# kubeflow/Code-Intelligence

Hardware: NVIDIA H100
Metric: issues/sec to 2400-d @ seq_len 512 batch 256 (higher is better)
Workload: dtype bf16

## Files before the change

code_intelligence_b200/_lib.py:

```python
from __future__ import annotations

import ctypes as C
import os
import subprocess
from pathlib import Path

_PKG = Path(__file__).resolve().parent
LIB_PATH = _PKG / "libissue_emb_b200.so"

IE_OK, IE_ERR_INVALID, IE_ERR_CUDA, IE_ERR_OOM, IE_ERR_STATE, IE_ERR_TOKEN = 0, -1, -2, -3, -4, -5
IE_FLAG_DEVICE_PTRS = 1
IE_MAX_BATCH = 3072
IE_CFG_ACCURATE_GATES, IE_CFG_FP32, IE_CFG_F32_GX = 1, 2, 4
IE_KNN_COSINE, IE_KNN_EUCLIDEAN = 0, 1


class ie_config(C.Structure):
    _fields_ = [("n_layers", C.c_int32), ("emb_sz", C.c_int32), ("n_hid", C.c_int32), ("vocab_sz", C.c_int32),
                ("pad_idx", C.c_int32), ("device", C.c_int32), ("flags", C.c_int32)]


PROTOTYPES = {
    "ie_version": (C.c_int, []),
    "ie_last_error": (C.c_char_p, []),
    "ie_encoder_create": (C.c_int, [C.POINTER(ie_config), C.POINTER(C.c_void_p)]),
    "ie_encoder_destroy": (None, [C.c_void_p]),
    "ie_encoder_load_embedding": (C.c_int, [C.c_void_p, C.c_void_p]),
    "ie_encoder_load_layer": (C.c_int, [C.c_void_p, C.c_int32, C.c_void_p, C.c_void_p, C.c_void_p, C.c_void_p]),
    "ie_encoder_encode": (C.c_int, [C.c_void_p, C.c_void_p, C.c_void_p, C.c_int32, C.c_int32, C.c_void_p, C.c_int32,
                                    C.c_void_p]),
    "ie_encoder_raw_features": (C.c_int, [C.c_void_p, C.c_void_p, C.c_int32, C.c_int32, C.c_void_p, C.c_int32,
                                          C.c_void_p]),
    "ie_encoder_launch_count": (C.c_int64, [C.c_void_p]),
    "ie_encoder_max_batch": (C.c_int32, [C.c_void_p]),
    "ie_encoder_check_errors": (C.c_int, [C.c_void_p]),
    "ie_encoder_last_phase_ms": (C.c_int, [C.c_void_p, C.c_void_p, C.c_int32]),
    "ie_encoder_last_phase_mhz": (C.c_int, [C.c_void_p, C.c_void_p, C.c_int32]),
    "ie_debug_seq_trace": (C.c_int64, [C.c_void_p, C.c_int32, C.c_void_p, C.c_int64]),
    "ie_mlp_create": (C.c_int, [C.c_int32, C.POINTER(C.c_int32), C.c_int32, C.POINTER(C.c_void_p)]),
    "ie_mlp_load_layer": (C.c_int, [C.c_void_p, C.c_int32, C.c_void_p, C.c_void_p]),
    "ie_mlp_predict_proba": (C.c_int, [C.c_void_p, C.c_void_p, C.c_int32, C.c_void_p, C.c_int32, C.c_void_p]),
    "ie_mlp_destroy": (None, [C.c_void_p]),
    "ie_pr_thresholds": (C.c_int, [C.c_void_p, C.c_void_p, C.c_int32, C.c_int32, C.c_double, C.c_double, C.c_void_p,
                                   C.c_void_p, C.c_void_p, C.c_int32, C.c_int32, C.c_void_p]),
    "ie_debug_gemm": (C.c_int, [C.c_void_p, C.c_void_p, C.c_void_p, C.c_int32, C.c_int32, C.c_int32, C.c_int32,
                                C.c_void_p, C.c_int32]),
    "ie_debug_gemm_ex": (C.c_int, [C.c_void_p, C.c_void_p, C.c_void_p, C.c_int32, C.c_int32, C.c_int32, C.c_int32,
                                   C.c_int32, C.c_int32, C.c_void_p, C.c_int32]),
    "ie_debug_gemm_frag": (C.c_int, [C.c_void_p, C.c_void_p, C.c_void_p, C.c_int32, C.c_int32, C.c_int32, C.c_int32,
                                     C.c_int32, C.c_void_p, C.c_int32]),
    "ie_debug_epilogue_layout": (C.c_int64, [C.c_int32, C.c_void_p, C.c_int64, C.c_void_p, C.c_void_p]),
    "ie_debug_layer_states": (C.c_int, [C.c_void_p, C.c_int32, C.c_void_p, C.c_int32, C.c_int32, C.c_void_p, C.c_int32,
                                        C.c_void_p]),
    "ie_knn_create": (C.c_int, [C.c_int32, C.c_int32, C.c_int32, C.POINTER(C.c_void_p)]),
    "ie_knn_destroy": (None, [C.c_void_p]),
    "ie_knn_add": (C.c_int, [C.c_void_p, C.c_void_p, C.c_int64, C.c_int32, C.c_void_p]),
    "ie_knn_search": (C.c_int, [C.c_void_p, C.c_void_p, C.c_int32, C.c_int32, C.c_void_p, C.c_void_p, C.c_int32,
                                C.c_void_p]),
    "ie_knn_check_errors": (C.c_int, [C.c_void_p]),
    "ie_debug_knn_shortlist": (C.c_int, [C.c_void_p, C.c_void_p, C.c_int32, C.c_int32, C.c_void_p, C.c_void_p]),
}

_lib = None


def build(verbose: bool = False) -> Path:
    r = subprocess.run(["make", "-C", str(_PKG / "csrc"), "-j8"], capture_output=True, text=True)
    if verbose or r.returncode != 0:
        print(r.stdout[-4000:])
        print(r.stderr[-4000:])
    if r.returncode != 0:
        raise RuntimeError("building libissue_emb_b200.so failed")
    return LIB_PATH


def load() -> C.CDLL:
    global _lib
    if _lib is not None:
        return _lib
    if not LIB_PATH.exists():
        if os.environ.get("IE_B200_NO_AUTOBUILD"):
            raise ImportError(f"{LIB_PATH} is missing (run `python -c 'import __graft_entry__ as g; g.build()'`)")
        build()
    lib = C.CDLL(str(LIB_PATH))
    for name, (res, args) in PROTOTYPES.items():
        fn = getattr(lib, name)
        fn.restype = res
        fn.argtypes = args
    _lib = lib
    return lib


def _debug_gemm(a, b, bias=None, act: int = 0, out_type: int = 0, segs: int = 1, device: int = 0):
    import numpy as np
    a = np.ascontiguousarray(a, dtype=np.float32)
    b = np.ascontiguousarray(b, dtype=np.float32)
    (M, K), N = a.shape, b.shape[0]
    if b.shape[1] != K:
        raise ValueError(f"a {a.shape} and b {b.shape} disagree on K")
    bias_p = None
    if bias is not None:
        bias = np.ascontiguousarray(bias, dtype=np.float32)
        if bias.shape != (N,):
            raise ValueError(f"bias {bias.shape} != ({N},)")
        bias_p = bias.ctypes.data
    d = np.empty((M, N), dtype=np.float32)
    check(load().ie_debug_gemm_ex(a.ctypes.data, b.ctypes.data, bias_p, M, N, K, act, out_type, segs, d.ctypes.data,
                                  device))
    return d


def check(rc: int) -> None:
    if rc == IE_OK:
        return
    msg = (load().ie_last_error() or b"").decode("utf-8", "replace")
    if rc in (IE_ERR_INVALID, IE_ERR_TOKEN):
        raise ValueError(msg)
    if rc == IE_ERR_OOM:
        raise RuntimeError("CUDA out of memory. " + msg)
    raise RuntimeError(msg)
```

code_intelligence_b200/csrc/api.cu:

```cuda
#include <algorithm>
#include <cmath>
#include <cstdarg>
#include <cstdio>
#include <cstdlib>
#include <cstring>
#include <mutex>
#include <string>
#include <vector>

#include <cuda_fp16.h>

#include "../../include/issue_emb_b200.h"
#include "kernels.h"

namespace {

thread_local std::string g_last_error;

int fail(int code, const char* fmt, ...) {
  char buf[512];
  va_list ap;
  va_start(ap, fmt);
  vsnprintf(buf, sizeof(buf), fmt, ap);
  va_end(ap);
// ... 934 lines not shown
  if (n16 >= 240 && n16 % 240 == 0) bn = 240;
  else if (n16 >= 128) bn = 128;
  else bn = n16;
  if (frag) bn = 256;
  const int n_pad = static_cast<int>(round_up(N, bn));
  const int ld = segs == 3 ? 2 * k_pad : k_pad;
  const size_t elt = out_type == 0 ? 4 : 2;
  DevBuf fa, fb, ba, bb, dd, db;
  cudaStream_t s = nullptr;
  CK(fa.reserve(static_cast<size_t>(M) * K * 4));
  CK(fb.reserve(static_cast<size_t>(N) * K * 4));
  CK(ba.reserve(static_cast<size_t>(m_pad) * ld * 2, true));
  CK(bb.reserve(static_cast<size_t>(n_pad) * ld * 2, true));
  CK(dd.reserve(static_cast<size_t>(m_pad) * n_pad * elt));
  CK(cudaMemcpy(fa.p, a, static_cast<size_t>(M) * K * 4, cudaMemcpyHostToDevice));
  CK(cudaMemcpy(fb.p, b, static_cast<size_t>(N) * K * 4, cudaMemcpyHostToDevice));
  const int lo_off = segs == 3 ? k_pad : 0;
  CK(ie::launch_convert_rows(fa.as<float>(), K, K, nullptr, M, ba.as<__nv_bfloat16>(), ld, lo_off, s));
  CK(ie::launch_convert_rows(fb.as<float>(), K, K, nullptr, N, bb.as<__nv_bfloat16>(), ld, lo_off, s));
  if (bias) {
    std::vector<float> bp(n_pad, 0.0f);
    if (frag) {
      for (int n = 0; n < N; ++n) bp[n / 256 * 256 + ie::frag_index(n % 256, 4)] = bias[n];
    } else {
      std::copy(bias, bias + N, bp.begin());
    }
    CK(db.reserve(n_pad * 4));
    CK(cudaMemcpy(db.p, bp.data(), n_pad * 4, cudaMemcpyHostToDevice));
  }
  ie::GemmArgs g{};
  g.a = ba.as<__nv_bfloat16>(); g.lda = ld;
  g.b = bb.as<__nv_bfloat16>(); g.ldb = ld;
  g.d = dd.p; g.ldd = n_pad;
  g.bias = bias ? db.as<float>() : nullptr;
  g.m_pad = m_pad; g.n_pad = n_pad; g.k_pad = k_pad;
  g.m_store = M; g.n_store = n_pad; g.bn = bn; g.act = act; g.out_bf16 = out_type; g.num_sms = sms; g.segs = segs;
  g.frag = frag ? 1 : 0;
  CK(ie::launch_gemm_bf16(g, s));
  if (frag) {
    std::vector<uint8_t> raw(static_cast<size_t>(M) * n_pad * elt);
    CK(cudaMemcpy(raw.data(), dd.p, raw.size(), cudaMemcpyDeviceToHost));
    for (size_t r = 0; r < static_cast<size_t>(M); ++r)
      for (int n = 0; n < N; ++n) {
        const size_t src = r * n_pad + n / 256 * 256 + ie::frag_index(n % 256, static_cast<int>(elt));
        if (out_type == 0) {
          std::memcpy(d + r * N + n, raw.data() + src * 4, 4);
        } else {
          __half_raw h;
          std::memcpy(&h.x, raw.data() + src * 2, 2);
          d[r * N + n] = __half2float(__half(h));
        }
      }
  } else if (out_type == 0) {
    CK(cudaMemcpy2D(d, static_cast<size_t>(N) * 4, dd.p, static_cast<size_t>(n_pad) * 4, static_cast<size_t>(N) * 4, M,
                    cudaMemcpyDeviceToHost));
  } else {
    std::vector<uint16_t> h16(static_cast<size_t>(M) * N);
    CK(cudaMemcpy2D(h16.data(), static_cast<size_t>(N) * 2, dd.p, static_cast<size_t>(n_pad) * 2, static_cast<size_t>(N) * 2,
                    M, cudaMemcpyDeviceToHost));
    for (size_t i = 0; i < h16.size(); ++i) {
      if (out_type == 1) {
        const uint32_t bits = static_cast<uint32_t>(h16[i]) << 16;
        std::memcpy(d + i, &bits, 4);
      } else {
        __half_raw r;
        r.x = h16[i];
        d[i] = __half2float(__half(r));
      }
    }
  }
  return IE_OK;
}

int ie_debug_gemm_ex(const float* a, const float* b, const float* bias, int32_t M, int32_t N, int32_t K, int32_t act,
                     int32_t out_type, int32_t segs, float* d, int32_t device) {
  return debug_gemm(a, b, bias, M, N, K, act, out_type, segs, d, device, false);
}

int ie_debug_gemm_frag(const float* a, const float* b, const float* bias, int32_t M, int32_t N, int32_t K, int32_t out_type,
                       int32_t segs, float* d, int32_t device) {
  return debug_gemm(a, b, bias, M, N, K, 0, out_type, segs, d, device, true);
}

int64_t ie_debug_epilogue_layout(int32_t out_units, int32_t* perm, int64_t cap, int32_t* frag2, int32_t* frag4) {
  if (out_units < 1) return fail(IE_ERR_INVALID, "out_units=%d must be >= 1", out_units);
  Layer L;
  L.out = out_units;
  L.out_pad = static_cast<int>(round_up(out_units, 64));
  const std::vector<int> p = slice_perm(L);
  if (perm != nullptr && cap >= static_cast<int64_t>(p.size())) std::copy(p.begin(), p.end(), perm);
  for (int c = 0; c < 256; ++c) {
    if (frag2 != nullptr) frag2[c] = ie::frag_index(c, 2);
    if (frag4 != nullptr) frag4[c] = ie::frag_index(c, 4);
  }
  return static_cast<int64_t>(p.size());
}

int ie_debug_gemm(const float* a, const float* b, const float* bias, int32_t M, int32_t N, int32_t K, int32_t act,
                  float* d, int32_t device) {
  return ie_debug_gemm_ex(a, b, bias, M, N, K, act, 0, 1, d, device);
}

}

struct ie_knn {
  int dim = 0, metric = IE_KNN_COSINE, device = 0, num_sms = 132;
  int k_pad = 0;
  long long n = 0, cap = 0;
  DevBuf xf;
  DevBuf xs;
  DevBuf col;
  DevBuf center;
  double c2 = 0.0;
  bool centred = false;
  DevBuf partial, qf, qs, rowt, cand, cnt, outd, outi, err;
  cudaStream_t own_stream = nullptr;
  cudaStream_t last_stream = nullptr;
  cudaEvent_t done_ev = nullptr;
  bool has_done = false;
  std::mutex mu;
};

namespace {

int knn_begin(ie_knn* h, bool dev, void* stream, cudaStream_t* s) {
  CK(cudaSetDevice(h->device));
  *s = (stream || dev) ? static_cast<cudaStream_t>(stream) : h->own_stream;
  if (h->has_done && *s != h->last_stream) CK(cudaStreamWaitEvent(*s, h->done_ev, 0));
  return IE_OK;
}

int knn_end(ie_knn* h, cudaStream_t s) {
  CK(cudaEventRecord(h->done_ev, s));
  h->last_stream = s;
  h->has_done = true;
  return IE_OK;
}

int knn_grow(DevBuf& b, size_t bytes, size_t keep, cudaStream_t s) {
  if (bytes <= b.cap) return IE_OK;
  DevBuf nb;
  CK(nb.reserve(bytes));
  if (keep) {
    CK(cudaMemcpyAsync(nb.p, b.p, keep, cudaMemcpyDeviceToDevice, s));
    CK(cudaStreamSynchronize(s));
  }
  b = std::move(nb);
  return IE_OK;
}

int knn_check_rows(const float* x, long long rows, int dim, const char* what) {
  for (long long r = 0; r < rows; ++r) {
    const float* v = x + r * dim;
    double s = 0.0;
    for (int i = 0; i < dim; ++i) {
      if (!std::isfinite(v[i]))
        return fail(IE_ERR_INVALID, "%s[%lld][%d] = %g is not finite", what, r, i, static_cast<double>(v[i]));
      s += static_cast<double>(v[i]) * v[i];
    }
    if (s > 0.0 && (s < ie::kKnnNormMin * ie::kKnnNormMin || s > ie::kKnnNormMax * ie::kKnnNormMax))
      return fail(IE_ERR_INVALID, "%s row %lld has norm %g, outside the index's range [2^-48, 2^48] (0 is allowed)",
                  what, r, std::sqrt(s));
  }
  return IE_OK;
}

// ... 194 lines not shown
```

code_intelligence_b200/csrc/gemm.cu:

```cuda
#include "gemm_kernel.cuh"

namespace ie {


cudaError_t launch_gemm_bf16(const GemmArgs& g, cudaStream_t stream) {
  if (g.m_pad % kBlockM || g.k_pad % kBlockK || g.bn % 16 || g.bn < 16 || g.bn > 256 || g.n_pad % g.bn ||
      g.n_store % 16 || g.ldd % 2)
    return cudaErrorInvalidValue;
  CUtensorMap tmA, tmB;
  const int segs = g.segs == 3 ? 3 : 1;
  const uint64_t k_inner = static_cast<uint64_t>(segs == 3 ? 2 : 1) * g.k_pad;
  const long long spin_limit = g.spin_limit > 0 ? g.spin_limit : kSpinLimitDefault;
  cudaError_t e = make_tmap_bf16_2d(&tmA, g.a, k_inner, g.m_pad, g.lda, kBlockK, kBlockM);
  if (e != cudaSuccess) return e;
  e = make_tmap_bf16_2d(&tmB, g.b, k_inner, g.n_pad, g.ldb, kBlockK, kBlockN);
  if (e != cudaSuccess) return e;

  const size_t smem = 1024 + static_cast<size_t>(kGemmStages) * kGemmStageBytes + 2 * kGemmStages * 8 + 32;
  const int num_m_blocks = g.m_pad / kBlockM;
  const int num_n_blocks = (g.n_pad + kBlockN - 1) / kBlockN;
  const int num_k_blocks = g.k_pad / kBlockK;
  const int num_tiles = num_m_blocks * num_n_blocks;
  const int sms = g.num_sms > 0 ? g.num_sms : 132;
  const int grid = num_tiles < sms ? num_tiles : sms;
  const int panel = 16;

#define IE_LAUNCH(OUT, ACT, FRAG)                                                                                  \
  do {                                                                                                             \
    auto kfn = gemm_bf16_kernel<OUT, ACT, FRAG>;                                                                       \
    e = cudaFuncSetAttribute(kfn, cudaFuncAttributeMaxDynamicSharedMemorySize, static_cast<int>(smem));            \
    if (e != cudaSuccess) return e;                                                                                \
    kfn<<<grid, kGemmThreads, smem, stream>>>(tmA, tmB, reinterpret_cast<OUT*>(g.d), g.bias, g.m_store, g.n_store, \
                                              g.ldd, num_m_blocks, num_n_blocks, num_k_blocks, panel, segs,        \
                                              g.k_pad, g.abort_flag, spin_limit, g.diag, DenseEpi{});              \
  } while (0)

  if (g.frag) {
    if (g.act != 0 || g.out_bf16 == 1 || g.bias == nullptr || g.n_store % kBlockN || g.n_store != g.n_pad ||
        (g.ldd * (g.out_bf16 == 2 ? 2 : 4)) % 16)
      return cudaErrorInvalidValue;
    if (g.out_bf16 == 2) IE_LAUNCH(__half, 0, true);
    else IE_LAUNCH(float, 0, true);
  } else if (g.out_bf16 == 2) {
    if (g.act != 0) return cudaErrorInvalidValue;
    IE_LAUNCH(__half, 0, false);
  } else if (g.out_bf16) {
    if (g.act == 0) IE_LAUNCH(__nv_bfloat16, 0, false);
    else if (g.act == 1) IE_LAUNCH(__nv_bfloat16, 1, false);
    else IE_LAUNCH(__nv_bfloat16, 2, false);
  } else {
    if (g.act == 0) IE_LAUNCH(float, 0, false);
    else if (g.act == 1) IE_LAUNCH(float, 1, false);
    else IE_LAUNCH(float, 2, false);
  }
#undef IE_LAUNCH
  return cudaGetLastError();
}

}
```

code_intelligence_b200/csrc/gemm_kernel.cuh:

```cuda
#pragma once
#include <cuda_fp16.h>
#include <type_traits>

#include "kernels.h"
#include "ptx.cuh"

namespace ie {

struct DenseEpi {
  static constexpr bool kSliced = false;
  static constexpr uint64_t kHintA = kEvictNormal;
  static constexpr uint64_t kHintB = kEvictLast;
  struct State {};
};

namespace {

__device__ __forceinline__ uint32_t pack_f16x2(float lo, float hi) {
  const __half2 v = __floats2half2_rn(lo, hi);
  return *reinterpret_cast<const uint32_t*>(&v);
}

constexpr int kBlockM = 128;
constexpr int kBlockN = 256;
constexpr int kBlockK = 64;
constexpr int kGemmThreads = 384;
constexpr int kGemmStages = 4;
constexpr uint32_t kABytes = kBlockM * kBlockK * 2;
constexpr uint32_t kBBytes = kBlockN * kBlockK * 2;
constexpr uint32_t kGemmStageBytes = kABytes + kBBytes;

template <typename OutT, int ACT, bool FRAG, typename Epi = DenseEpi>
__global__ void __launch_bounds__(kGemmThreads, 1)
gemm_bf16_kernel(const __grid_constant__ CUtensorMap tmA, const __grid_constant__ CUtensorMap tmB, OutT* __restrict__ D,
                 const float* __restrict__ bias, int m_store, int n_store, long long ldd, int num_m_blocks,
                 int num_n_blocks, int num_k_blocks, int panel, int segs, int k_pad, unsigned* abort_flag,
                 long long spin_limit, long long* diag, const __grid_constant__ Epi epi) {
  extern __shared__ uint8_t smem_raw[];
  const uint32_t raw = smem_u32(smem_raw);
  uint8_t* smem = smem_raw + ((1024u - (raw & 1023u)) & 1023u);

  uint64_t* full_bar = reinterpret_cast<uint64_t*>(smem + kGemmStages * kGemmStageBytes);
  uint64_t* empty_bar = full_bar + kGemmStages;
  uint32_t* abort_s = reinterpret_cast<uint32_t*>(empty_bar + kGemmStages);
  const Abort ab{abort_s, abort_flag, spin_limit};
  const int nkt = num_k_blocks * segs;

  const int warp = threadIdx.x >> 5;
  const int lane = threadIdx.x & 31;

  if (warp == 0 && lane == 0) {
    tma_prefetch_desc(&tmA);
    tma_prefetch_desc(&tmB);
    if (diag != nullptr && blockIdx.x == 0) {
      unsigned long long g;
      asm volatile("mov.u64 %0, %%globaltimer;" : "=l"(g));
      diag[0] = clock64();
      diag[1] = static_cast<long long>(g);
    }
  }
  if (warp == 1 && lane == 0) {
    for (int s = 0; s < kGemmStages; ++s) {
      mbar_init(&full_bar[s], 1);
      mbar_init(&empty_bar[s], 2);
    }
    *abort_s = 0;
    fence_barrier_init();
  }
  __syncthreads();

  int num_tiles = num_m_blocks * num_n_blocks;
  if constexpr (Epi::kSliced) num_tiles = epi.num_tiles();
  const int panel_tiles = panel * num_n_blocks;
  int first_tile = blockIdx.x;
  if constexpr (Epi::kSliced) first_tile = epi.first_tile(blockIdx.x);
  auto next_tile = [&](int tile) {
    if constexpr (Epi::kSliced) return epi.next_tile(tile, gridDim.x, num_n_blocks);
    else return tile + static_cast<int>(gridDim.x);
  };
  auto decode = [&](int tile, int& m_blk, int& n_blk) {
    if constexpr (Epi::kSliced) {
      epi.decode(tile, num_m_blocks, m_blk, n_blk);
      return;
    }
    const int p = tile / panel_tiles;
    const int r = tile - p * panel_tiles;
    const int m0 = p * panel;
    const int mcnt = min(panel, num_m_blocks - m0);
    n_blk = r / mcnt;
    m_blk = m0 + (r - n_blk * mcnt);
  };

  if (warp < 4) {
    if (warp == 0 && lane == 0) {
      int stage = 0;
      uint32_t phase = 0;
      for (int tile = first_tile; tile < num_tiles && !aborted(ab); tile = next_tile(tile)) {
        int m_blk, n_blk;
        decode(tile, m_blk, n_blk);
        for (int kb = 0; kb < nkt; ++kb) {
          const int seg = kb / num_k_blocks, r = kb - seg * num_k_blocks;
          mbar_wait(&empty_bar[stage], phase ^ 1, ab);
          uint8_t* sa = smem + static_cast<size_t>(stage) * kGemmStageBytes;
          mbar_arrive_expect_tx(&full_bar[stage], kGemmStageBytes);
          tma_load_2d(sa, &tmA, &full_bar[stage], (seg == 1 ? k_pad : 0) + r * kBlockK, m_blk * kBlockM, Epi::kHintA);
          tma_load_2d(sa + kABytes, &tmB, &full_bar[stage], (seg == 2 ? k_pad : 0) + r * kBlockK, n_blk * kBlockN,
                      Epi::kHintB);
          if (++stage == kGemmStages) { stage = 0; phase ^= 1; }
        }
      }
    }
  } else {
    const int wg = (warp - 4) >> 2;
    const int q = lane & 3;
    const int rbase = wg * 64 + (warp & 3) * 16 + (lane >> 2);
    const uint32_t smem_base = smem_u32(smem);
    const bool signal = (threadIdx.x & 127) == 0;
    int stage = 0;
    uint32_t phase = 0;
    float d[128];
    typename Epi::State st{};
    for (int tile = first_tile; tile < num_tiles; tile = next_tile(tile)) {
      int m_blk, n_blk;
      decode(tile, m_blk, n_blk);
      int prev = -1;
      for (int kb = 0; kb < nkt; ++kb) {
        mbar_wait(&full_bar[stage], phase, ab);
        const uint32_t sa = smem_base + stage * kGemmStageBytes;
        const uint64_t da = wgmma_desc_sw128(sa + wg * (kABytes / 2));
        const uint64_t db = wgmma_desc_sw128(sa + kABytes);
        wgmma_fence();
#pragma unroll
        for (int k = 0; k < kBlockK / 16; ++k) wgmma_m64n256k16(d, da + 2 * k, db + 2 * k, (kb | k) != 0);
        wgmma_commit();
        if (prev >= 0) {
          wgmma_wait<1>();
          if (signal) mbar_arrive(&empty_bar[prev]);
        }
        prev = stage;
        if (++stage == kGemmStages) { stage = 0; phase ^= 1; }
      }
      wgmma_wait<0>();
      wgmma_fence_regs(d);
      if (signal && prev >= 0) mbar_arrive(&empty_bar[prev]);
      if constexpr (Epi::kSliced) {
        epi.tile(d, m_blk, n_blk, wg * 64 + (warp & 3) * 16, lane, st);
        continue;
      }
      if constexpr (FRAG) {
        constexpr int kPer = 16 / static_cast<int>(sizeof(OutT));
        const float4* bq = reinterpret_cast<const float4*>(bias) + n_blk * (kBlockN / 4) + q;
        OutT* drow[2];
#pragma unroll
        for (int hr = 0; hr < 2; ++hr)
          drow[hr] = D + static_cast<long long>(m_blk * kBlockM + rbase + 8 * hr) * ldd + n_blk * kBlockN + q * kPer;
#pragma unroll
        for (int k = 0; k < 64 / kPer; ++k) {
          float4 b[kPer / 4];
#pragma unroll
          for (int i = 0; i < kPer / 4; ++i) b[i] = __ldg(bq + 4 * (k * (kPer / 4) + i));
#pragma unroll
          for (int hr = 0; hr < 2; ++hr) {
            if (m_blk * kBlockM + rbase + 8 * hr >= m_store) continue;
            float x[kPer];
#pragma unroll
            for (int i = 0; i < kPer / 4; ++i) {
              const int m = k * (kPer / 4) + i;
              x[4 * i + 0] = d[8 * m + 2 * hr] + b[i].x;
              x[4 * i + 1] = d[8 * m + 2 * hr + 1] + b[i].y;
              x[4 * i + 2] = d[8 * m + 4 + 2 * hr] + b[i].z;
              x[4 * i + 3] = d[8 * m + 4 + 2 * hr + 1] + b[i].w;
            }
            uint4 v;
            if constexpr (sizeof(OutT) == 4) {
              v = make_uint4(__float_as_uint(x[0]), __float_as_uint(x[1]), __float_as_uint(x[2]), __float_as_uint(x[3]));
            } else {
              v = make_uint4(pack_f16x2(x[0], x[1]), pack_f16x2(x[2], x[3]), pack_f16x2(x[4], x[5]), pack_f16x2(x[6], x[7]));
            }
            *reinterpret_cast<uint4*>(drow[hr] + 4 * k * kPer) = v;
          }
        }
        continue;
      }
#pragma unroll
      for (int hr = 0; hr < 2; ++hr) {
        const int row = m_blk * kBlockM + rbase + 8 * hr;
        if (row >= m_store) continue;
        OutT* drow = D + static_cast<long long>(row) * ldd;
#pragma unroll
        for (int jg = 0; jg < kBlockN / 8; ++jg) {
          const int n = n_blk * kBlockN + 8 * jg + 2 * q;
          if (n < n_store) {
            float x0 = d[4 * jg + 2 * hr], x1 = d[4 * jg + 2 * hr + 1];
            if (bias != nullptr) {
              const float2 b2 = __ldg(reinterpret_cast<const float2*>(bias + n));
              x0 += b2.x;
              x1 += b2.y;
            }
            if (ACT == 1) { x0 = fmaxf(x0, 0.0f); x1 = fmaxf(x1, 0.0f); }
            if (ACT == 2) { x0 = sigmoid_acc(x0); x1 = sigmoid_acc(x1); }
            if constexpr (sizeof(OutT) == 4) {
              *reinterpret_cast<float2*>(drow + n) = make_float2(x0, x1);
            } else if constexpr (std::is_same<OutT, __half>::value) {
              *reinterpret_cast<uint32_t*>(drow + n) = pack_f16x2(x0, x1);
            } else {
              *reinterpret_cast<uint32_t*>(drow + n) = pack_bf16x2(x0, x1);
            }
          }
        }
      }
    }
    if constexpr (Epi::kSliced) epi.finish(wg * 64 + (warp & 3) * 16, lane, st);
  }

  __syncwarp();
  if (diag != nullptr && threadIdx.x == 128 && blockIdx.x == 0) {
    unsigned long long g;
    asm volatile("mov.u64 %0, %%globaltimer;" : "=l"(g));
    diag[2] = clock64();
    diag[3] = static_cast<long long>(g);
  }
}

}

}
```

code_intelligence_b200/csrc/kernels.h:

```cpp
#pragma once
#include <cuda.h>
#include <cuda_bf16.h>
#include <cuda_runtime.h>
#include <stddef.h>
#include <stdint.h>

namespace ie {

cudaError_t make_tmap_bf16_2d(CUtensorMap* out, const void* base, uint64_t inner, uint64_t rows, uint64_t ld,
                              uint32_t box_inner, uint32_t box_rows);

__host__ __device__ inline int frag_index(int c, int elem_bytes) {
  const int q = (c & 7) >> 1;
  const int ix = 4 * (c >> 4) + 2 * ((c >> 3) & 1) + (c & 1);
  const int per_chunk = 16 / elem_bytes;
  return (ix / per_chunk * 4 + q) * per_chunk + ix % per_chunk;
}

struct GemmArgs {
  const __nv_bfloat16* a;
  const __nv_bfloat16* b;
  void* d;
  const float* bias;
  int m_pad, n_pad, k_pad;
  long long lda, ldb, ldd;
  int m_store, n_store;
  int bn;
  int act;
  int out_bf16;
  int num_sms;
  int segs;
  unsigned* abort_flag;
  long long spin_limit;
  long long* diag;
  int frag;
};
cudaError_t launch_gemm_bf16(const GemmArgs& g, cudaStream_t stream);

constexpr int kMaxBatches = 12;
struct LstmLayerArgs {
  CUtensorMap tm_h;
  CUtensorMap tm_w;
  CUtensorMap tm_h64;
  CUtensorMap tm_x;
  int pre_nkb;
  const float* bias;
  int mc;
  int mc_ctas;
  const void* gx;
  const int* tok;
  float* c;
  __nv_bfloat16* y;
  float* raw;
  float* pool_sum;
  float* pool_max;
  float* pool_last;
  const int* lengths;
  unsigned* step_done;
  unsigned* abort_flag;
  long long spin_limit;
  int T, t0, T_total;
  int single_step;
  int t_step;
  int ng;
  int u, n_cta, out_pad, kh_pad;
  long long ldy, raw_ld;
  int gate_mode, gx_bf16, segs;
  int num_sms, check_only, cooperative;
  int fault;
  long long* trace;
  int trace_items;
  long long* diag;
};
cudaError_t launch_lstm_layer(const LstmLayerArgs& a, cudaStream_t stream);
int lstm_layer_ctas(const LstmLayerArgs& a);
int lstm_layer_max_ctas();

cudaError_t launch_embed_gather(const int64_t* ids, int B, int T, int b_pad, const __nv_bfloat16* emb, int vocab,
                                int e_pad, __nv_bfloat16* x0, long long ldx, int pad_idx, int* err_flag, int t0, int Tc,
                                cudaStream_t stream);
cudaError_t launch_prep_lengths(const int* lengths_in, int B, int T, int b_pad, int* lengths_out, int* err_flag,
                                cudaStream_t stream);
cudaError_t launch_tokens_time_major(const int64_t* ids, int B, int T, int b_pad, int vocab, int pad_idx, int* tok,
                                     int* err_flag, cudaStream_t stream);
cudaError_t launch_pool_finalize(const float* pool_sum, const float* pool_max, const float* pool_last,
                                 const int* lengths, int B, int e, int out_pad, float* out, cudaStream_t stream);
cudaError_t launch_convert_rows(const float* src, long long ld_src, int cols, const int* perm, int rows_dst,
                                __nv_bfloat16* dst, long long ld_dst, int lo_off, cudaStream_t stream);
cudaError_t launch_fill_f32(float* p, size_t n, float v, cudaStream_t stream);

constexpr int kPrMaxSamples = 16384;
cudaError_t launch_pr_thresholds(const float* scores, const uint8_t* truth, int n, int n_labels, double p_thr,
                                 double r_thr, float* out_thr, double* out_prec, double* out_rec, cudaStream_t stream);

constexpr int kKnnCap = 512;
constexpr int kKnnMergeMax = 16384;
constexpr int kKnnExtra = 32;
constexpr double kKnnNormMin = 0x1p-48, kKnnNormMax = 0x1p48;
size_t knn_center_workspace(int D);
cudaError_t launch_knn_center(const float* x, long long n, int D, int k_pad, double* partial, float* center,
                              cudaStream_t stream);
cudaError_t launch_knn_prep(const float* src, long long rows, long long rows_pad, int D, int k_pad, const float* center,
                            double c2, int mode, __nv_bfloat16* dst, float2* terms, int* err, cudaStream_t stream);
void knn_plan(int nq, long long n, int kp, int num_sms, int* S, int* nbs);
struct KnnStage1Args {
  const __nv_bfloat16* qs;
  const __nv_bfloat16* xs;
  const float2* col;
  const float2* rowt;
  uint2* cand;
  int* cnt;
  long long n;
  int nq, m_pad, k_pad, S, nbs, kp, cosine, num_sms;
};
cudaError_t launch_knn_stage1(const KnnStage1Args& a, cudaStream_t stream);
cudaError_t launch_knn_merge_rerank(const uint2* cand, const int* cnt, int rows, int S, int kp, const float* Q,
                                    const float* X, int D, int cosine, int k, float* out_dist, int64_t* out_idx,
                                    float* dbg_score, int64_t* dbg_idx, cudaStream_t stream);
// ... 3 lines not shown
```

code_intelligence_b200/csrc/knn.cu:

```cuda
#include <algorithm>

#include "gemm_kernel.cuh"

namespace ie {

namespace {

__device__ __forceinline__ uint32_t order_key(float s) {
  const uint32_t b = __float_as_uint(s) == 0x80000000u ? 0u : __float_as_uint(s);
  return (b & 0x80000000u) ? ~b : (b | 0x80000000u);
}
__device__ __forceinline__ float key_score(uint32_t k) {
  return __uint_as_float((k & 0x80000000u) ? (k & 0x7fffffffu) : ~k);
}

__device__ __noinline__ float knn_compact(uint2* buf, int count, int kp, int lane) {
  __syncwarp();
  uint32_t t = 0;
  for (int bit = 31; bit >= 0; --bit) {
    const uint32_t c = t | (1u << bit);
    int m = 0;
    for (int i = lane; i < count; i += 32) m += buf[i].x >= c;
    if (static_cast<int>(__reduce_add_sync(~0u, static_cast<unsigned>(m))) >= kp) t = c;
  }
// ... 332 lines not shown
        }
      } else {
        double s = 0.0;
        for (int i = lane; i < D; i += 32) {
          const double t = static_cast<double>(q[i]) - static_cast<double>(x[i]);
          s += t * t;
        }
        dist = sqrt(warp_sum(s));
      }
    }
    if (lane == 0) { cd[j] = dist; ci[j] = idx; }
  }
  __syncthreads();
  for (int t = threadIdx.x; t < kp; t += blockDim.x) {
    int rank = 0;
    for (int j = 0; j < kp; ++j) rank += (cd[j] < cd[t]) || (cd[j] == cd[t] && ci[j] < ci[t]);
    if (rank < k) {
      out_dist[static_cast<size_t>(row) * k + rank] = static_cast<float>(cd[t]);
      out_idx[static_cast<size_t>(row) * k + rank] = ci[t];
    }
  }
}

constexpr int kCenterChunks = 256;

}

size_t knn_center_workspace(int D) { return static_cast<size_t>(kCenterChunks) * D * sizeof(double); }

cudaError_t launch_knn_center(const float* x, long long n, int D, int k_pad, double* partial, float* center,
                              cudaStream_t stream) {
  const long long per = (n + kCenterChunks - 1) / kCenterChunks;
  const int chunks = static_cast<int>((n + per - 1) / per);
  knn_center_partial_kernel<<<dim3((D + 127) / 128, chunks), 128, 0, stream>>>(x, n, D, per, partial);
  knn_center_finish_kernel<<<(k_pad + 127) / 128, 128, 0, stream>>>(partial, chunks, n, D, k_pad, center);
  return cudaGetLastError();
}

cudaError_t launch_knn_prep(const float* src, long long rows, long long rows_pad, int D, int k_pad, const float* center,
                            double c2, int mode, __nv_bfloat16* dst, float2* terms, int* err, cudaStream_t stream) {
  if (rows_pad < 1 || rows_pad > 0x7fffffffll) return cudaErrorInvalidValue;
  knn_prep_rows_kernel<<<static_cast<unsigned>(rows_pad), 256, 0, stream>>>(src, rows, D, k_pad, center, c2, mode, dst,
                                                                            terms, err);
  return cudaGetLastError();
}

void knn_plan(int nq, long long n, int kp, int num_sms, int* S, int* nbs) {
  const int m_blocks = (nq + 127) / 128;
  const long long n_blocks = (n + 255) / 256;
  long long s = std::max(1, num_sms / m_blocks);
  s = std::min<long long>(s, n_blocks);
  s = std::min<long long>(s, kKnnMergeMax / kp);
  *nbs = static_cast<int>((n_blocks + s - 1) / s);
  *S = static_cast<int>((n_blocks + *nbs - 1) / *nbs);
}

cudaError_t launch_knn_stage1(const KnnStage1Args& a, cudaStream_t stream) {
  if (a.m_pad % 128 || a.k_pad % 64 || a.nq > a.m_pad) return cudaErrorInvalidValue;
  CUtensorMap tmA, tmB;
  cudaError_t e = make_tmap_bf16_2d(&tmA, a.qs, 2ull * a.k_pad, a.m_pad, 2ull * a.k_pad, kBlockK, kBlockM);
  if (e != cudaSuccess) return e;
  e = make_tmap_bf16_2d(&tmB, a.xs, 2ull * a.k_pad, static_cast<uint64_t>(a.n), 2ull * a.k_pad, kBlockK, kBlockN);
  if (e != cudaSuccess) return e;
  KnnEpi epi{};
  epi.cand = a.cand;
  epi.cnt = a.cnt;
  epi.col = a.col;
  epi.rowt = a.rowt;
  epi.nq = a.nq;
  epi.n = static_cast<int>(a.n);
  epi.S = a.S;
  epi.nbs = a.nbs;
  epi.kp = a.kp;
  epi.cosine = a.cosine;
  epi.m_blocks = a.m_pad / kBlockM;
  epi.items = epi.m_blocks * a.S;
  const int num_n_blocks = static_cast<int>((a.n + kBlockN - 1) / kBlockN);
  const int grid = std::min(epi.items, a.num_sms > 0 ? a.num_sms : 132);
  const size_t smem = 1024 + static_cast<size_t>(kGemmStages) * kGemmStageBytes + 2 * kGemmStages * 8 + 32;
  auto kfn = gemm_bf16_kernel<float, 0, false, KnnEpi>;
  e = cudaFuncSetAttribute(kfn, cudaFuncAttributeMaxDynamicSharedMemorySize, static_cast<int>(smem));
  if (e != cudaSuccess) return e;
  kfn<<<grid, kGemmThreads, smem, stream>>>(tmA, tmB, nullptr, nullptr, 0, 0, 0, epi.m_blocks, num_n_blocks,
                                            a.k_pad / kBlockK, 16, 3, a.k_pad, nullptr, kSpinLimitDefault, nullptr, epi);
  return cudaGetLastError();
}

cudaError_t launch_knn_merge_rerank(const uint2* cand, const int* cnt, int rows, int S, int kp, const float* Q,
                                    const float* X, int D, int cosine, int k, float* out_dist, int64_t* out_idx,
                                    float* dbg_score, int64_t* dbg_idx, cudaStream_t stream) {
  int P = 1;
  while (P < S * kp) P <<= 1;
  const size_t smem = static_cast<size_t>(P) * 8 + static_cast<size_t>(kp) * 16;
  auto kfn = knn_merge_rerank_kernel;
  cudaError_t e = cudaFuncSetAttribute(kfn, cudaFuncAttributeMaxDynamicSharedMemorySize, static_cast<int>(smem));
  if (e != cudaSuccess) return e;
  kfn<<<rows, 512, smem, stream>>>(cand, cnt, S, kp, P, Q, X, D, cosine, k, out_dist, out_idx, dbg_score, dbg_idx);
  return cudaGetLastError();
}

}
```

include/issue_emb_b200.h:

```cpp
#ifndef ISSUE_EMB_B200_H_
#define ISSUE_EMB_B200_H_

#include <stdint.h>

#ifdef __cplusplus
extern "C" {
#endif

#define IE_OK 0
#define IE_ERR_INVALID (-1)
#define IE_ERR_CUDA (-2)
#define IE_ERR_OOM (-3)
#define IE_ERR_STATE (-4)
#define IE_ERR_TOKEN (-5)

#define IE_FLAG_DEVICE_PTRS 1

#define IE_CFG_ACCURATE_GATES 1
#define IE_CFG_FP32 2
#define IE_CFG_F32_GX 4

#define IE_MAX_BATCH 3072

typedef struct ie_encoder ie_encoder;
typedef struct ie_mlp ie_mlp;

typedef struct ie_config {
  int32_t n_layers;
  int32_t emb_sz;
  int32_t n_hid;
  int32_t vocab_sz;
  int32_t pad_idx;
  int32_t device;
  int32_t flags;
} ie_config;

int ie_version(void);
const char* ie_last_error(void);

int ie_encoder_create(const ie_config* cfg, ie_encoder** out);
void ie_encoder_destroy(ie_encoder* h);

int ie_encoder_load_embedding(ie_encoder* h, const float* emb);
int ie_encoder_load_layer(ie_encoder* h, int32_t layer, const float* w_ih, const float* w_hh, const float* b_ih,
                          const float* b_hh);

int ie_encoder_encode(ie_encoder* h, const int64_t* ids, const int32_t* lengths, int32_t B, int32_t T, float* out,
                      int32_t flags, void* stream);

int ie_encoder_raw_features(ie_encoder* h, const int64_t* ids, int32_t B, int32_t T, float* raw, int32_t flags,
                            void* stream);

int64_t ie_encoder_launch_count(const ie_encoder* h);

int32_t ie_encoder_max_batch(const ie_encoder* h);

int ie_encoder_check_errors(ie_encoder* h);

int ie_encoder_last_phase_ms(ie_encoder* h, float* ms, int32_t cap);

int ie_encoder_last_phase_mhz(ie_encoder* h, float* mhz, int32_t cap);

int64_t ie_debug_seq_trace(ie_encoder* h, int32_t layer, long long* out, int64_t cap);

int ie_mlp_create(int32_t n_layers, const int32_t* dims, int32_t device, ie_mlp** out);
int ie_mlp_load_layer(ie_mlp* m, int32_t layer, const float* coef, const float* intercept);
int ie_mlp_predict_proba(ie_mlp* m, const float* X, int32_t n, float* probs, int32_t flags, void* stream);
void ie_mlp_destroy(ie_mlp* m);

int ie_pr_thresholds(const float* scores, const uint8_t* truth, int32_t n, int32_t n_labels, double precision_threshold,
                     double recall_threshold, float* thresholds, double* precisions, double* recalls, int32_t device,
                     int32_t flags, void* stream);

int ie_debug_gemm(const float* a, const float* b, const float* bias, int32_t M, int32_t N, int32_t K, int32_t act,
                  float* d, int32_t device);

int ie_debug_gemm_ex(const float* a, const float* b, const float* bias, int32_t M, int32_t N, int32_t K, int32_t act,
                     int32_t out_type, int32_t segs, float* d, int32_t device);

int ie_debug_gemm_frag(const float* a, const float* b, const float* bias, int32_t M, int32_t N, int32_t K,
                       int32_t out_type, int32_t segs, float* d, int32_t device);

int64_t ie_debug_epilogue_layout(int32_t out_units, int32_t* perm, int64_t cap, int32_t* frag2, int32_t* frag4);

int ie_debug_layer_states(ie_encoder* h, int32_t layer, const int64_t* ids, int32_t B, int32_t T, float* out,
                          int32_t flags, void* stream);

#define IE_KNN_COSINE 0
#define IE_KNN_EUCLIDEAN 1
typedef struct ie_knn ie_knn;
int ie_knn_create(int32_t dim, int32_t metric, int32_t device, ie_knn** out);
void ie_knn_destroy(ie_knn* h);
int ie_knn_add(ie_knn* h, const float* X, int64_t n, int32_t flags, void* stream);
int ie_knn_search(ie_knn* h, const float* Q, int32_t nq, int32_t k, float* dist, int64_t* idx, int32_t flags,
                  void* stream);
int ie_knn_check_errors(ie_knn* h);
int ie_debug_knn_shortlist(ie_knn* h, const float* Q, int32_t nq, int32_t k, float* score, int64_t* idx);

#ifdef __cplusplus
}
#endif
#endif
```

Baseline: 4200.

## Overlap GEMM epilogue stores with next tile's mainloop and rebalance warp registers

For the 16-bit fragment epilogue, the consumer now packs bias-added results into registers and defers the global stores, issuing them between the first few k-block WGMMAs of the next tile. Bias is prefetched a few k-blocks before the mainloop ends, and setmaxnreg moves registers from producer warps to consumer warps. The aim is to hide epilogue store latency behind tensor-core work, at the cost of extra live registers (pk, bv) that could spill. The change also adds globaltimer tracing hooks and a device-pointer debug GEMM entry point.

```diff
diff --git a/code_intelligence_b200/_lib.py b/code_intelligence_b200/_lib.py
--- a/code_intelligence_b200/_lib.py
+++ b/code_intelligence_b200/_lib.py
@@ -49,6 +49,8 @@
                                    C.c_int32, C.c_int32, C.c_void_p, C.c_int32]),
     "ie_debug_gemm_frag": (C.c_int, [C.c_void_p, C.c_void_p, C.c_void_p, C.c_int32, C.c_int32, C.c_int32, C.c_int32,
                                      C.c_int32, C.c_void_p, C.c_int32]),
+    "ie_debug_gemm_device": (C.c_int, [C.c_void_p, C.c_void_p, C.c_void_p, C.c_void_p, C.c_int32, C.c_int32, C.c_int32,
+                                       C.c_int32, C.c_int32, C.c_void_p, C.c_int32, C.c_void_p, C.c_int32]),
     "ie_debug_epilogue_layout": (C.c_int64, [C.c_int32, C.c_void_p, C.c_int64, C.c_void_p, C.c_void_p]),
     "ie_debug_layer_states": (C.c_int, [C.c_void_p, C.c_int32, C.c_void_p, C.c_int32, C.c_int32, C.c_void_p, C.c_int32,
                                         C.c_void_p]),
diff --git a/code_intelligence_b200/csrc/api.cu b/code_intelligence_b200/csrc/api.cu
--- a/code_intelligence_b200/csrc/api.cu
+++ b/code_intelligence_b200/csrc/api.cu
@@ -1040,6 +1040,26 @@
   return debug_gemm(a, b, bias, M, N, K, 0, out_type, segs, d, device, true);
 }
 
+int ie_debug_gemm_device(const void* a, const void* b, const float* bias, void* d, int32_t M, int32_t N, int32_t K,
+                         int32_t out_type, int32_t frag, long long* trace, int32_t trace_tiles, long long* diag,
+                         int32_t device) {
+  if (a == nullptr || b == nullptr || bias == nullptr || d == nullptr || M < 128 || M % 128 || N < 256 || N % 256 ||
+      K < 64 || K % 64 || (out_type != 0 && out_type != 2) || (frag != 0 && frag != 1) || trace_tiles < 0)
+    return fail(IE_ERR_INVALID, "bad argument");
+  CK(cudaSetDevice(device));
+  int sms = 132;
+  CK(cudaDeviceGetAttribute(&sms, cudaDevAttrMultiProcessorCount, device));
+  ie::GemmArgs g{};
+  g.a = static_cast<const __nv_bfloat16*>(a); g.lda = K;
+  g.b = static_cast<const __nv_bfloat16*>(b); g.ldb = K;
+  g.d = d; g.ldd = N; g.bias = bias;
+  g.m_pad = M; g.n_pad = N; g.k_pad = K;
+  g.m_store = M; g.n_store = N; g.bn = 256; g.act = 0; g.out_bf16 = out_type; g.num_sms = sms; g.segs = 1;
+  g.frag = frag; g.diag = diag; g.trace = trace; g.trace_tiles = trace != nullptr ? trace_tiles : 0;
+  CK(ie::launch_gemm_bf16(g, nullptr));
+  return IE_OK;
+}
+
 int64_t ie_debug_epilogue_layout(int32_t out_units, int32_t* perm, int64_t cap, int32_t* frag2, int32_t* frag4) {
   if (out_units < 1) return fail(IE_ERR_INVALID, "out_units=%d must be >= 1", out_units);
   Layer L;
diff --git a/code_intelligence_b200/csrc/gemm.cu b/code_intelligence_b200/csrc/gemm.cu
--- a/code_intelligence_b200/csrc/gemm.cu
+++ b/code_intelligence_b200/csrc/gemm.cu
@@ -32,7 +32,8 @@
     if (e != cudaSuccess) return e;                                                                                \
     kfn<<<grid, kGemmThreads, smem, stream>>>(tmA, tmB, reinterpret_cast<OUT*>(g.d), g.bias, g.m_store, g.n_store, \
                                               g.ldd, num_m_blocks, num_n_blocks, num_k_blocks, panel, segs,        \
-                                              g.k_pad, g.abort_flag, spin_limit, g.diag, DenseEpi{});              \
+                                              g.k_pad, g.abort_flag, spin_limit, g.diag, g.trace, g.trace_tiles,   \
+                                              DenseEpi{});                                                         \
   } while (0)
 
   if (g.frag) {
diff --git a/code_intelligence_b200/csrc/gemm_kernel.cuh b/code_intelligence_b200/csrc/gemm_kernel.cuh
--- a/code_intelligence_b200/csrc/gemm_kernel.cuh
+++ b/code_intelligence_b200/csrc/gemm_kernel.cuh
@@ -29,13 +29,28 @@
 constexpr uint32_t kABytes = kBlockM * kBlockK * 2;
 constexpr uint32_t kBBytes = kBlockN * kBlockK * 2;
 constexpr uint32_t kGemmStageBytes = kABytes + kBBytes;
+constexpr uint32_t kGemmProducerRegs = 40;
+constexpr uint32_t kGemmConsumerRegs = 232;
+static_assert(128 * kGemmProducerRegs + 256 * kGemmConsumerRegs <= kGemmThreads * 168,
+              "setmaxnreg budgets exceed the launch's registers");
+constexpr int kBiasAhead = 4;
+constexpr int kStoreBlocks = 4;
+
+__device__ __forceinline__ void gemm_trace(long long* trace, int trace_tiles, int k, int slot) {
+  if (trace != nullptr && k < trace_tiles) {
+    unsigned long long g;
+    asm volatile("mov.u64 %0, %%globaltimer;" : "=l"(g));
+    trace[(static_cast<long long>(blockIdx.x) * trace_tiles + k) * 4 + slot] = static_cast<long long>(g);
+  }
+}
 
 template <typename OutT, int ACT, bool FRAG, typename Epi = DenseEpi>
 __global__ void __launch_bounds__(kGemmThreads, 1)
 gemm_bf16_kernel(const __grid_constant__ CUtensorMap tmA, const __grid_constant__ CUtensorMap tmB, OutT* __restrict__ D,
                  const float* __restrict__ bias, int m_store, int n_store, long long ldd, int num_m_blocks,
                  int num_n_blocks, int num_k_blocks, int panel, int segs, int k_pad, unsigned* abort_flag,
-                 long long spin_limit, long long* diag, const __grid_constant__ Epi epi) {
+                 long long spin_limit, long long* diag, long long* trace, int trace_tiles,
+                 const __grid_constant__ Epi epi) {
   extern __shared__ uint8_t smem_raw[];
   const uint32_t raw = smem_u32(smem_raw);
   uint8_t* smem = smem_raw + ((1024u - (raw & 1023u)) & 1023u);
@@ -92,6 +107,7 @@
   };
 
   if (warp < 4) {
+    setmaxnreg_dec<kGemmProducerRegs>();
     if (warp == 0 && lane == 0) {
       int stage = 0;
       uint32_t phase = 0;
@@ -111,21 +127,44 @@
       }
     }
   } else {
+    setmaxnreg_inc<kGemmConsumerRegs>();
     const int wg = (warp - 4) >> 2;
     const int q = lane & 3;
     const int rbase = wg * 64 + (warp & 3) * 16 + (lane >> 2);
     const uint32_t smem_base = smem_u32(smem);
     const bool signal = (threadIdx.x & 127) == 0;
+    const bool tracer = trace != nullptr && threadIdx.x == 128;
     int stage = 0;
     uint32_t phase = 0;
     float d[128];
     typename Epi::State st{};
-    for (int tile = first_tile; tile < num_tiles; tile = next_tile(tile)) {
+    constexpr bool kOverlap = FRAG && sizeof(OutT) == 2;
+    float4 bv[16];
+    uint32_t pk[64];
+    OutT* pend[2] = {nullptr, nullptr};
+    auto store_chunk = [&](int k) {
+#pragma unroll
+      for (int hr = 0; hr < 2; ++hr)
+        if (pend[hr] != nullptr)
+          *reinterpret_cast<uint4*>(pend[hr] + 32 * k) =
+              make_uint4(pk[32 * hr + 4 * k], pk[32 * hr + 4 * k + 1], pk[32 * hr + 4 * k + 2], pk[32 * hr + 4 * k + 3]);
+    };
+    auto store_rest = [&](int k0, int k_done) {
+#pragma unroll
+      for (int k = k0; k < 8; ++k) store_chunk(k);
+      pend[0] = pend[1] = nullptr;
+      if (tracer && k_done >= 0) gemm_trace(trace, trace_tiles, k_done, 3);
+    };
+    const int kpeel = nkt < kStoreBlocks ? nkt : kStoreBlocks;
+    const int kb_bias = nkt - kBiasAhead > kpeel ? nkt - kBiasAhead : kpeel;
+    int kt = 0;
+    for (int tile = first_tile; tile < num_tiles; tile = next_tile(tile), ++kt) {
       int m_blk, n_blk;
       decode(tile, m_blk, n_blk);
       int prev = -1;
-      for (int kb = 0; kb < nkt; ++kb) {
+      auto kblock = [&](int kb, auto between) {
         mbar_wait(&full_bar[stage], phase, ab);
+        if (tracer && kb == 0) gemm_trace(trace, trace_tiles, kt, 0);
         const uint32_t sa = smem_base + stage * kGemmStageBytes;
         const uint64_t da = wgmma_desc_sw128(sa + wg * (kABytes / 2));
         const uint64_t db = wgmma_desc_sw128(sa + kABytes);
@@ -133,53 +172,78 @@
 #pragma unroll
         for (int k = 0; k < kBlockK / 16; ++k) wgmma_m64n256k16(d, da + 2 * k, db + 2 * k, (kb | k) != 0);
         wgmma_commit();
+        between();
         if (prev >= 0) {
           wgmma_wait<1>();
           if (signal) mbar_arrive(&empty_bar[prev]);
         }
         prev = stage;
         if (++stage == kGemmStages) { stage = 0; phase ^= 1; }
+      };
+      auto nothing = [] {};
+      if constexpr (kOverlap) {
+#pragma unroll
+        for (int j = 0; j < kStoreBlocks; ++j) {
+          if (j < kpeel) {
+            kblock(j, [&] {
+              store_chunk(2 * j);
+              store_chunk(2 * j + 1);
+              if (j + 1 == kpeel) store_rest(2 * j + 2, kt - 1);
+            });
+          }
+        }
+        int kb = kpeel;
+        for (; kb < kb_bias; ++kb) kblock(kb, nothing);
+        const float4* bq = reinterpret_cast<const float4*>(bias) + n_blk * (kBlockN / 4) + q;
+#pragma unroll
+        for (int m = 0; m < 16; ++m) bv[m] = __ldg(bq + 4 * m);
+        for (; kb < nkt; ++kb) kblock(kb, nothing);
+      } else {
+        for (int kb = 0; kb < nkt; ++kb) kblock(kb, nothing);
       }
       wgmma_wait<0>();
       wgmma_fence_regs(d);
+      if (tracer) gemm_trace(trace, trace_tiles, kt, 1);
       if (signal && prev >= 0) mbar_arrive(&empty_bar[prev]);
       if constexpr (Epi::kSliced) {
         epi.tile(d, m_blk, n_blk, wg * 64 + (warp & 3) * 16, lane, st);
         continue;
       }
+      if constexpr (kOverlap) {
+#pragma unroll
+        for (int m = 0; m < 16; ++m) {
+#pragma unroll
+          for (int hr = 0; hr < 2; ++hr) {
+            pk[32 * hr + 2 * m] = pack_f16x2(d[8 * m + 2 * hr] + bv[m].x, d[8 * m + 2 * hr + 1] + bv[m].y);
+            pk[32 * hr + 2 * m + 1] = pack_f16x2(d[8 * m + 4 + 2 * hr] + bv[m].z, d[8 * m + 4 + 2 * hr + 1] + bv[m].w);
+          }
+        }
+#pragma unroll
+        for (int hr = 0; hr < 2; ++hr) {
+          const int row = m_blk * kBlockM + rbase + 8 * hr;
+          pend[hr] = row < m_store ? D + static_cast<long long>(row) * ldd + n_blk * kBlockN + q * 8 : nullptr;
+        }
+        if (tracer) gemm_trace(trace, trace_tiles, kt, 2);
+        continue;
+      }
       if constexpr (FRAG) {
-        constexpr int kPer = 16 / static_cast<int>(sizeof(OutT));
         const float4* bq = reinterpret_cast<const float4*>(bias) + n_blk * (kBlockN / 4) + q;
         OutT* drow[2];
 #pragma unroll
         for (int hr = 0; hr < 2; ++hr)
-          drow[hr] = D + static_cast<long long>(m_blk * kBlockM + rbase + 8 * hr) * ldd + n_blk * kBlockN + q * kPer;
-#pragma unroll
-        for (int k = 0; k < 64 / kPer; ++k) {
-          float4 b[kPer / 4];
-#pragma unroll
-          for (int i = 0; i < kPer / 4; ++i) b[i] = __ldg(bq + 4 * (k * (kPer / 4) + i));
+          drow[hr] = D + static_cast<long long>(m_blk * kBlockM + rbase + 8 * hr) * ldd + n_blk * kBlockN + q * 4;
+#pragma unroll
+        for (int m = 0; m < 16; ++m) {
+          const float4 b = __ldg(bq + 4 * m);
 #pragma unroll
           for (int hr = 0; hr < 2; ++hr) {
             if (m_blk * kBlockM + rbase + 8 * hr >= m_store) continue;
-            float x[kPer];
-#pragma unroll
-            for (int i = 0; i < kPer / 4; ++i) {
-              const int m = k * (kPer / 4) + i;
-              x[4 * i + 0] = d[8 * m + 2 * hr] + b[i].x;
-              x[4 * i + 1] = d[8 * m + 2 * hr + 1] + b[i].y;
-              x[4 * i + 2] = d[8 * m + 4 + 2 * hr] + b[i].z;
-              x[4 * i + 3] = d[8 * m + 4 + 2 * hr + 1] + b[i].w;
-            }
-            uint4 v;
-            if constexpr (sizeof(OutT) == 4) {
-              v = make_uint4(__float_as_uint(x[0]), __float_as_uint(x[1]), __float_as_uint(x[2]), __float_as_uint(x[3]));
-            } else {
-              v = make_uint4(pack_f16x2(x[0], x[1]), pack_f16x2(x[2], x[3]), pack_f16x2(x[4], x[5]), pack_f16x2(x[6], x[7]));
-            }
-            *reinterpret_cast<uint4*>(drow[hr] + 4 * k * kPer) = v;
-          }
-        }
+            *reinterpret_cast<float4*>(drow[hr] + 16 * m) =
+                make_float4(d[8 * m + 2 * hr] + b.x, d[8 * m + 2 * hr + 1] + b.y, d[8 * m + 4 + 2 * hr] + b.z,
+                            d[8 * m + 4 + 2 * hr + 1] + b.w);
+          }
+        }
+        if (tracer) { gemm_trace(trace, trace_tiles, kt, 2); gemm_trace(trace, trace_tiles, kt, 3); }
         continue;
       }
 #pragma unroll
@@ -210,6 +274,7 @@
         }
       }
     }
+    if constexpr (kOverlap) store_rest(0, kt - 1);
     if constexpr (Epi::kSliced) epi.finish(wg * 64 + (warp & 3) * 16, lane, st);
   }
 
diff --git a/code_intelligence_b200/csrc/kernels.h b/code_intelligence_b200/csrc/kernels.h
--- a/code_intelligence_b200/csrc/kernels.h
+++ b/code_intelligence_b200/csrc/kernels.h
@@ -34,6 +34,8 @@
   long long spin_limit;
   long long* diag;
   int frag;
+  long long* trace;
+  int trace_tiles;
 };
 cudaError_t launch_gemm_bf16(const GemmArgs& g, cudaStream_t stream);
 
diff --git a/code_intelligence_b200/csrc/knn.cu b/code_intelligence_b200/csrc/knn.cu
--- a/code_intelligence_b200/csrc/knn.cu
+++ b/code_intelligence_b200/csrc/knn.cu
@@ -438,7 +438,7 @@
   e = cudaFuncSetAttribute(kfn, cudaFuncAttributeMaxDynamicSharedMemorySize, static_cast<int>(smem));
   if (e != cudaSuccess) return e;
   kfn<<<grid, kGemmThreads, smem, stream>>>(tmA, tmB, nullptr, nullptr, 0, 0, 0, epi.m_blocks, num_n_blocks,
-                                            a.k_pad / kBlockK, 16, 3, a.k_pad, nullptr, kSpinLimitDefault, nullptr, epi);
+                                            a.k_pad / kBlockK, 16, 3, a.k_pad, nullptr, kSpinLimitDefault, nullptr, nullptr, 0, epi);
   return cudaGetLastError();
 }
 
diff --git a/include/issue_emb_b200.h b/include/issue_emb_b200.h
--- a/include/issue_emb_b200.h
+++ b/include/issue_emb_b200.h
@@ -81,6 +81,10 @@
 int ie_debug_gemm_frag(const float* a, const float* b, const float* bias, int32_t M, int32_t N, int32_t K,
                        int32_t out_type, int32_t segs, float* d, int32_t device);
 
+int ie_debug_gemm_device(const void* a, const void* b, const float* bias, void* d, int32_t M, int32_t N, int32_t K,
+                         int32_t out_type, int32_t frag, long long* trace, int32_t trace_tiles, long long* diag,
+                         int32_t device);
+
 int64_t ie_debug_epilogue_layout(int32_t out_units, int32_t* perm, int64_t cap, int32_t* frag2, int32_t* frag4);
 
 int ie_debug_layer_states(ie_encoder* h, int32_t layer, const int64_t* ids, int32_t B, int32_t T, float* out,
```

Result: faster. 4289 (median of 6 runs) (+2.1%).
